# citiususc/veryfasttree

Measured on AMD Instinct MI355X. Metric: profile-ops/sec, higher is better.
Workload: dtype f32; 1 GPU; c4_1M_x200_nt_tophits; n_seqs=1000000, n_pos=200, active_nodes=750000, top_k=2000

## Files before the change

veryfasttree_amd/csrc/vft_api.hip:

```cpp
#include <hip/hip_runtime.h>
#include <csignal>
#include <unistd.h>

#include <cmath>
#include <cstdarg>
#include <cstdio>
#include <cstdlib>
#include <cstring>
#include <new>
#include <algorithm>
#include <utility>
#include <vector>
#include <chrono>

#include "../../include/vft_hip.h"
#include "vft_owned.h"
#include "vft_staging.h"
#define VFT_PAIR_STAGE_CAP 2048
#include "vft_kernels_ml.h"

VFT_ML_HEAVY_INSTANCES(extern)
#include "vft_kernels_ml_long.h"
VFT_ML_LONG_INSTANCES(extern)
#include "vft_kernels_nj.h"
// ... 2231 lines not shown
        c->slots[(size_t) profPos[q]].nPart = (int) gridP;
    }
    a.M.L.mq = nullptr;
    a.M.L.lq = (const uint32_t *) lq;
    a.M.P.mq = (const REAL *) mq;
    a.M.P.lq = nullptr;
    kernel_event(c);
    launch((k_sweep_nt_mixed_multi<REAL, S, S>), dim3((unsigned) (a.nInt + nLeafWGs)), dim3(VFT_WG), 0, c->stream, a);
    kernel_event(c);
    kernel_event(c);
    if (c->timeKernels) c->kevSweeps += 2 * S - 1;
    LAUNCHCHK(c);
    return VFT_OK;
}

static int no_slot(vft_ctx *c) { return fail(c, VFT_ERR_STATE, "the context has no sweep buffers (vft_create failed)"); }

static int sweep_args_ok(vft_ctx *c, int64_t query, int64_t nActive, int32_t k) {
    if (c->slots.empty()) return no_slot(c);
    if (!c->leavesUp) return fail(c, VFT_ERR_STATE, "vft_sweep before vft_upload_leaves");
    if (query < 0 || query >= c->maxnode || nActive < 3 || k < 0 || k > c->hitsCap)
        return fail(c, VFT_ERR_INVALID, "vft_sweep: bad arguments (query %lld, nActive %lld, k %d)", (long long) query,
                    (long long) nActive, (int) k);
    return VFT_OK;
}

extern "C" int vft_sweep(vft_ctx *c, int64_t query, int64_t nActive, int64_t nDiffAllow, double totdiam, int32_t k,
                         void *hits, void *dHitsOut, int64_t *bestJ) {
    if (!c) return VFT_ERR_INVALID;
    if (int r = sweep_args_ok(c, query, nActive, k)) return r;
    if (int r = sweep_one(c, 0, query, nActive, nDiffAllow, totdiam)) return r;
    if (k == 0) return VFT_OK;
    if (bestJ && k < 2) return fail(c, VFT_ERR_INVALID, "vft_sweep: best_j needs k >= 2");
    const int64_t lo = c->shardLo, hi = c->shardHi < c->maxnode ? c->shardHi : c->maxnode;
    int r;
    if (c->cfg.precision == 4) r = run_select<float, vft_hit_f32>(c, 1, &query, lo, hi, k);
    else r = run_select<double, vft_hit_f64>(c, 1, &query, lo, hi, k);
    if (r) return r;
    const size_t hb = (size_t) k * (c->cfg.precision == 4 ? sizeof(vft_hit_f32) : sizeof(vft_hit_f64));
    const vft_ctx::SweepSlotHost &h = c->slots[0];
    if (dHitsOut) HIPCHK(c, hipMemcpyAsync(dHitsOut, h.dRes + sizeof(SelectHeader), hb, hipMemcpyDeviceToDevice, c->stream));
    if (hits) memcpy(hits, h.hRes + sizeof(SelectHeader), hb);
    if (bestJ) *bestJ = (int64_t) ((const SelectHeader *) h.hRes)->bestJ;
    return VFT_OK;
}

struct SeedGroup {
    int pos[4];
    int n;
    bool leaf;
};

extern "C" int vft_sweep_batch(vft_ctx *c, int32_t nSeeds, const int64_t *queries, int64_t nActive, int64_t nDiffAllow,
                               double totdiam, int32_t k, void *hits, void *dHitsOut, int64_t *bestJ) {
    if (!c || !queries || nSeeds < 1 || nSeeds > VFT_MAX_SLOTS || k < 1) return VFT_ERR_INVALID;
    if (bestJ && k < 2) return fail(c, VFT_ERR_INVALID, "vft_sweep_batch: best_j needs k >= 2");
    for (int s = 0; s < nSeeds; s++)
        if (int r = sweep_args_ok(c, queries[s], nActive, k)) return r;
    if (int r = ensure_slots(c, nSeeds)) return r;
    const bool staged = c->cfg.n_codes == 4 && !c->hasDm && nSeeds > 1;
    std::vector<SeedGroup> groups;
    if (staged && !c->noMultiSweep && !(c->maxStamp - nActive > nDiffAllow)) {
        bool fresh = true;
        for (int s = 0; s < nSeeds && fresh; s++) fresh = !((int64_t) c->hNOut[queries[s]] - nActive > nDiffAllow);
        const int maxGroup = c->multiMax ? c->multiMax : 4;
        for (int kind = 0; kind < 2 && fresh; kind++) {
            SeedGroup g{};
            g.leaf = kind == 0;
            int nLeft = 0;
            auto isKind = [&](int s) { return (queries[s] < c->d.nSeqs) == (kind == 0); };
            for (int s = 0; s < nSeeds; s++) nLeft += isKind(s);
            for (int s = 0; s < nSeeds; s++) {
                if (!isKind(s)) continue;
                g.pos[g.n++] = s;
                nLeft--;
                if (g.n == maxGroup || (g.n == 2 && nLeft < 2)) {
                    groups.push_back(g);
                    g.n = 0;
                }
            }
        }
    }
    const int64_t nPosPad = (int64_t) c->d.nChunk * VFT_CHUNK;
    const size_t mqGroupBytes = (size_t) nPosPad * VFT_MQ_STRIDE(4) * c->rs;
    const size_t lqGroupBytes = (size_t) nPosPad * sizeof(uint32_t);
    if (!groups.empty() && !c->mqBuf) {
        OWNCHK(own_group(c, [&]() -> int {
            OWNCHK(own_dev(c, &c->mqBuf, 32 * mqGroupBytes));
            return own_dev(c, &c->lqBuf, 32 * lqGroupBytes);
        }));
        c->mqGroupBytes = mqGroupBytes;
        c->lqGroupBytes = lqGroupBytes;
    }
    if (staged) {
        if (int r = flush_pending(c)) return r;
        std::vector<int> mqGroup((size_t) nSeeds, -1), mqIdx((size_t) nSeeds, 0), mqS((size_t) nSeeds, 0), lqGroup((size_t) nSeeds, -1);
        for (size_t g = 0; g < groups.size(); g++)
            for (int q = 0; q < groups[g].n; q++) {
                (groups[g].leaf ? lqGroup : mqGroup)[(size_t) groups[g].pos[q]] = (int) g;
                mqIdx[(size_t) groups[g].pos[q]] = q;
                mqS[(size_t) groups[g].pos[q]] = groups[g].n;
            }
        Stage st;
        if (int r = st.open(c, (size_t) nSeeds * (c->cfg.precision == 4 ? sizeof(QuerySlot<float>) : sizeof(QuerySlot<double>)), Stage::RING_ONLY)) return r;
        if (c->cfg.precision == 4) {
            for (int s = 0; s < nSeeds; s++) {
                QuerySlot<float> qs;
                qs.node = queries[s];
                qs.q = qbuf_slot<float>(c, s);
                qs.mq = mqGroup[(size_t) s] >= 0 ? (float *) ((char *) c->mqBuf + (size_t) mqGroup[(size_t) s] * c->mqGroupBytes) : nullptr;
                qs.lq = lqGroup[(size_t) s] >= 0 ? (uint32_t *) ((char *) c->lqBuf + (size_t) lqGroup[(size_t) s] * c->lqGroupBytes) : nullptr;
                qs.mqIdx = qs.lqIdx = mqIdx[(size_t) s];
                qs.mqS = qs.lqS = mqS[(size_t) s];
                st.put((size_t) s * sizeof(qs), &qs, sizeof(qs));
            }
            launch((k_extract_query_batch<float, 4>), dim3(cdiv(nPosPad, 256), (unsigned) nSeeds), dim3(256), 0, c->stream, arena<float>(c), st.dev<const QuerySlot<float>>(0));
        } else {
            for (int s = 0; s < nSeeds; s++) {
                QuerySlot<double> qs;
                qs.node = queries[s];
                qs.q = qbuf_slot<double>(c, s);
                qs.mq = mqGroup[(size_t) s] >= 0 ? (double *) ((char *) c->mqBuf + (size_t) mqGroup[(size_t) s] * c->mqGroupBytes) : nullptr;
                qs.lq = lqGroup[(size_t) s] >= 0 ? (uint32_t *) ((char *) c->lqBuf + (size_t) lqGroup[(size_t) s] * c->lqGroupBytes) : nullptr;
                qs.mqIdx = qs.lqIdx = mqIdx[(size_t) s];
                qs.mqS = qs.lqS = mqS[(size_t) s];
                st.put((size_t) s * sizeof(qs), &qs, sizeof(qs));
            }
            launch((k_extract_query_batch<double, 4>), dim3(cdiv(nPosPad, 256), (unsigned) nSeeds), dim3(256), 0, c->stream, arena<double>(c), st.dev<const QuerySlot<double>>(0));
        }
        LAUNCHCHK(c);
    }
    std::vector<char> done((size_t) nSeeds, 0);
    std::vector<char> groupDone(groups.size(), 0);
    if (c->cfg.precision == 4 && !c->noMixedSweep && !groups.empty() && mixed_sweep_fits(c)) {
        size_t gl = 0, gp = 0;
        for (;;) {
            while (gl < groups.size() && !(groups[gl].leaf && groups[gl].n == 4)) gl++;
            while (gp < groups.size() && !(!groups[gp].leaf && groups[gp].n == 4)) gp++;
            if (gl == groups.size() || gp == groups.size()) break;
            const void *mq = (const void *) ((char *) c->mqBuf + gp * c->mqGroupBytes);
            const void *lq = (const void *) ((char *) c->lqBuf + gl * c->lqGroupBytes);
            if (int r = sweep_mixed<float>(c, groups[gl].pos, groups[gp].pos, queries, nActive, nDiffAllow, totdiam, mq, lq)) return r;
            for (int q = 0; q < 4; q++) done[(size_t) groups[gl].pos[q]] = done[(size_t) groups[gp].pos[q]] = 1;
            groupDone[gl++] = groupDone[gp++] = 1;
        }
    }
    for (size_t g = 0; g < groups.size(); g++) {
        if (groupDone[g]) continue;
        const SeedGroup &G = groups[g];
        const void *mq = G.leaf ? nullptr : (const void *) ((char *) c->mqBuf + g * c->mqGroupBytes);
        const void *lq = G.leaf ? (const void *) ((char *) c->lqBuf + g * c->lqGroupBytes) : nullptr;
        int r;
        if (c->cfg.precision == 4) r = G.n == 4 ? sweep_group<float, 4>(c, G.leaf, G.pos, queries, nActive, nDiffAllow, totdiam, mq, lq) : sweep_group<float, 2>(c, G.leaf, G.pos, queries, nActive, nDiffAllow, totdiam, mq, lq);
        else r = G.n == 4 ? sweep_group<double, 4>(c, G.leaf, G.pos, queries, nActive, nDiffAllow, totdiam, mq, lq) : sweep_group<double, 2>(c, G.leaf, G.pos, queries, nActive, nDiffAllow, totdiam, mq, lq);
        if (r) return r;
        for (int q = 0; q < G.n; q++) done[(size_t) G.pos[q]] = 1;
    }
    for (int s = 0; s < nSeeds; s++)
        if (!done[(size_t) s])
            if (int r = sweep_one(c, s, queries[s], nActive, nDiffAllow, totdiam, staged)) return r;
    const int64_t lo = c->shardLo, hi = c->shardHi < c->maxnode ? c->shardHi : c->maxnode;
    int r;
    if (c->cfg.precision == 4) r = run_select<float, vft_hit_f32>(c, nSeeds, queries, lo, hi, k);
    else r = run_select<double, vft_hit_f64>(c, nSeeds, queries, lo, hi, k);
    if (r) return r;
    const size_t hb = (size_t) k * (c->cfg.precision == 4 ? sizeof(vft_hit_f32) : sizeof(vft_hit_f64));
    for (int s = 0; s < nSeeds; s++) {
// ... 1900 lines not shown
```

veryfasttree_amd/csrc/vft_kernels_nj.h:

```cpp
#pragma once
#include "vft_device.h"

#define VFT_WG 256

template <typename REAL>
struct QueryBuf {
    REAL *w;
    uint8_t *code;
    REAL *f;
    uint4 *enc;
    double2 *tab;
};

template <typename REAL>
__device__ __forceinline__ void vft_query_tab(const QueryBuf<REAL> &q, int64_t p, REAL wq, const REAL *f) {
#pragma unroll
    for (int c = 0; c < 5; c++) {
        double2 v = make_double2(0.0, 0.0);
        if (c < 4 && wq > 0) {
            const double wgt = (double) wq;
            const double piece = 1.0 - (double) f[c < 4 ? c : 0];
            v = make_double2(wgt * piece, wgt);
        }
        q.tab[p * 5 + c] = v;
    }
}

template <typename REAL, int NC>
__device__ __forceinline__ void vft_extract_query(const Arena<REAL> &A, int64_t node, const QueryBuf<REAL> &q) {
    const int64_t p = (int64_t) blockIdx.x * blockDim.x + threadIdx.x;
    const int64_t nPosPad = (int64_t) A.d.nChunk * VFT_CHUNK;
    if (p >= nPosPad) return;
    REAL w = 0;
    int code = VFT_NOCODE_;
    REAL f[NC];
#pragma unroll
    for (int k = 0; k < NC; k++) f[k] = 0;
    if (p < A.d.nPos) {
        Col<REAL, NC> c;
        vft_load_col<REAL, NC>(A, node, p, c);
        w = c.w;
        code = c.code;
        if (c.vec) {
#pragma unroll
            for (int k = 0; k < NC; k++) f[k] = c.f[k];
        } else if (NC == 4 && code != VFT_NOCODE_) {
#pragma unroll
            for (int k = 0; k < NC; k++) f[k] = (k == code) ? (REAL) 1 : (REAL) 0;
        }
    }
    q.w[p] = w;
    q.code[p] = (uint8_t) code;
#pragma unroll
    for (int k = 0; k < NC; k++) q.f[p * NC + k] = f[k];
    if (NC == 4) vft_query_tab<REAL>(q, p, w, f);
    if (node < A.d.nSeqs && p < A.d.nChunk) {
        q.enc[p] = A.leafT[vft_leaf_idx(A.d, node >> 6, (int) p, (int) (node & 63))];
    }
}
template <typename REAL, int NC>
__global__ void k_extract_query(Arena<REAL> A, int64_t node, QueryBuf<REAL> q) {
    vft_extract_query<REAL, NC>(A, node, q);
}
#ifdef VFT_NO_PLAIN_COLUMNS
#define VFT_PLAIN_COLUMNS 0
#define VFT_MQ_STRIDE(S) (4 * (S) + 4)
#else
#define VFT_PLAIN_COLUMNS 1
#define VFT_MQ_STRIDE(S) (4 * (S) + 8)
#endif
#ifdef VFT_NO_SEED_CODE_RECORDS
#define VFT_SEED_CODE_RECORDS 0
#else
#define VFT_SEED_CODE_RECORDS 1
#endif
#if defined(VFT_NO_GPR_INDEX_SELECT) || !VFT_SEED_CODE_RECORDS || !VFT_PLAIN_COLUMNS
#define VFT_GPR_INDEX_SELECT 0
#else
#define VFT_GPR_INDEX_SELECT 1
#endif
#if defined(VFT_NO_SHARED_PIECES) || !VFT_GPR_INDEX_SELECT
#define VFT_SHARED_PIECES 0
#else
#define VFT_SHARED_PIECES 1
#endif
template <typename REAL>
struct QuerySlot {
    int64_t node;
    QueryBuf<REAL> q;
    REAL *mq;
    int32_t mqIdx, mqS;
    uint32_t *lq;
    int32_t lqIdx, lqS;
};
template <typename REAL, int NC>
__global__ void k_extract_query_batch(Arena<REAL> A, const QuerySlot<REAL> *qs) {
    const QuerySlot<REAL> &sl = qs[blockIdx.y];
    vft_extract_query<REAL, NC>(A, sl.node, sl.q);
    if (VFT_SEED_CODE_RECORDS && NC == 4 && sl.lq) {
        const int64_t p = (int64_t) blockIdx.x * blockDim.x + threadIdx.x;
        if (p < (int64_t) A.d.nChunk * VFT_CHUNK) {
            uint8_t *dst = (uint8_t *) (sl.lq + p);
            dst[sl.lqIdx] = sl.q.code[p];
            if (sl.lqIdx == 0)
                for (int k = sl.lqS; k < 4; k++) dst[k] = VFT_NOCODE_;
        }
    }
    if (NC == 4 && sl.mq) {
        const int64_t p = (int64_t) blockIdx.x * blockDim.x + threadIdx.x;
        if (p < (int64_t) A.d.nChunk * VFT_CHUNK) {
            REAL *dst = sl.mq + p * VFT_MQ_STRIDE(sl.mqS);
#pragma unroll
            for (int k = 0; k < 4; k++) dst[4 * sl.mqIdx + k] = sl.q.f[p * 4 + k];
            dst[4 * sl.mqS + sl.mqIdx] = sl.q.w[p];
            if (VFT_PLAIN_COLUMNS) ((uint8_t *) (dst + 4 * sl.mqS + 4))[sl.mqIdx] = sl.q.code[p];
        }
    }
}

template <typename REAL, int NC>
__global__ void k_outprofile_as_query(Arena<REAL> A, QueryBuf<REAL> q) {
    const int64_t p = (int64_t) blockIdx.x * blockDim.x + threadIdx.x;
    const int64_t nPosPad = (int64_t) A.d.nChunk * VFT_CHUNK;
    if (p >= nPosPad) return;
    const bool in = p < A.d.nPos;
    q.w[p] = in ? A.outW[p] : (REAL) 0;
    q.code[p] = VFT_NOCODE_;
    REAL f[NC];
#pragma unroll
    for (int k = 0; k < NC; k++) {
        f[k] = in ? A.outF[p * NC + k] : (REAL) 0;
        q.f[p * NC + k] = f[k];
    }
    if (NC == 4) vft_query_tab<REAL>(q, p, in ? A.outW[p] : (REAL) 0, f);
}

struct SweepArgs {
    int64_t query;
    int64_t lo, hi;
    int64_t nActive, nDiffAllow;
    double totdiam;
    int32_t queryIsLeaf;
    int32_t force;
    int32_t nLeafWG;
    int32_t pad;
    int64_t leafEnd;
    int64_t heavyLo;
};

template <typename REAL>
struct SweepOut {
    REAL *dist, *weight, *crit;
    REAL *partMin, *partMax;
};

template <typename REAL, int NWAVES>
__device__ __forceinline__ void vft_block_minmax_n(REAL cmin, REAL cmax, REAL *partMin, REAL *partMax, int part) {
    __shared__ REAL smin[NWAVES], smax[NWAVES];
#pragma unroll
    for (int off = 32; off > 0; off >>= 1) {
        const REAL a = __shfl_xor(cmin, off, 64), b = __shfl_xor(cmax, off, 64);
        cmin = a < cmin ? a : cmin;
        cmax = b > cmax ? b : cmax;
    }
    if ((threadIdx.x & 63) == 0) {
        smin[threadIdx.x >> 6] = cmin;
        smax[threadIdx.x >> 6] = cmax;
    }
    __syncthreads();
    if (threadIdx.x == 0) {
#pragma unroll
        for (int w = 1; w < NWAVES; w++) {
            cmin = smin[w] < cmin ? smin[w] : cmin;
            cmax = smax[w] > cmax ? smax[w] : cmax;
        }
        partMin[part] = cmin;
        partMax[part] = cmax;
    }
}
template <typename REAL>
__device__ __forceinline__ void vft_block_minmax(REAL cmin, REAL cmax, REAL *partMin, REAL *partMax, int part) {
    vft_block_minmax_n<REAL, VFT_WG / 64>(cmin, cmax, partMin, partMax, part);
}

enum { MODE_CRIT = 0, MODE_OUTDIST = 1, MODE_CRIT_LEAFQ = 2 };

__device__ __forceinline__ void vft_seq_counts(const uint4 a, const uint4 b, int &nUse, int &nSame) {
    const uint32_t x = a.x & b.x, y = a.y & b.y, z = a.z & b.z, w = a.w & b.w;
    nUse += __popc(x & 0x10101010u) + __popc(y & 0x10101010u) + __popc(z & 0x10101010u) + __popc(w & 0x10101010u);
    nSame += __popc(x & 0x0F0F0F0Fu) + __popc(y & 0x0F0F0F0Fu) + __popc(z & 0x0F0F0F0Fu) + __popc(w & 0x0F0F0F0Fu);
}

__device__ __forceinline__ void vft_seq_counts_packed(const uint4 a, const uint4 b, uint32_t &cnt) {
    const uint32_t x = a.x & b.x, y = a.y & b.y, z = a.z & b.z, w = a.w & b.w;
    const uint32_t same = __popc(x & 0x0F0F0F0Fu) + __popc(y & 0x0F0F0F0Fu) + __popc(z & 0x0F0F0F0Fu) + __popc(w & 0x0F0F0F0Fu);
    cnt += __popc(x & 0x10101010u) + __popc(y & 0x10101010u) + __popc(z & 0x10101010u) + __popc(w & 0x10101010u);
    cnt += same << 16;
}
// ... 862 lines not shown
        for (int q = 0; q < GC; q++)
#pragma unroll
            for (int bt = 0; bt < NBT; bt++)
#pragma unroll
                for (int sd = 0; sd < S; sd++) {
                    denom[bt][sd] += v[bt][q][sd].y;
                    top[bt][sd] += v[bt][q][sd].x;
                }
    }
}

template <int SL>
struct LeafEncChunk {
    uint4 e[SL > 0 ? SL : 1];
};
template <int SL>
__device__ __forceinline__ void vft_leaf_enc_load(LeafEncChunk<SL> &d, const uint4 *const *enc, int c) {
    typedef uint32_t __attribute__((ext_vector_type(4))) u4_t;
    typedef const __attribute__((address_space(4))) u4_t *cp_t;
#pragma unroll
    for (int q = 0; q < SL; q++) {
        const u4_t v = *((cp_t) enc[q] + c);
        d.e[q] = make_uint4(v.x, v.y, v.z, v.w);
    }
}
template <int NBT, int S, int SL>
__device__ __forceinline__ void vft_leaf_walk_chunk(const double2 *row, const uint4 *t, double (*top)[S], double (*denom)[S],
                                                    const LeafEncChunk<SL> &e, uint32_t (*cnt)[SL > 0 ? SL : 1]) {
    if constexpr (SL > 0) {
#pragma unroll
        for (int bt = 0; bt < NBT; bt++) vft_leaf_table_chunk_multi<1, S, 1>(row, t + bt, top + bt, denom + bt);
        __builtin_amdgcn_sched_barrier(0);
#pragma unroll
        for (int bt = 0; bt < NBT; bt++)
#pragma unroll
            for (int q = 0; q < SL; q++) vft_seq_counts_packed(t[bt], e.e[q], cnt[bt][q]);
    } else {
        vft_leaf_table_chunk_multi<NBT, S>(row, t, top, denom);
    }
}

template <typename REAL, int NBT, int S, int SL = 0>
__device__ __forceinline__ void vft_leaf_table_walk_multi(const Arena<REAL> &A, const MultiLeafQ<REAL, S> &M, double2 *tab, const int64_t *tj,
                                                          double (*top)[S], double (*denom)[S], const uint4 *const *enc = nullptr,
                                                          uint32_t (*cnt)[SL > 0 ? SL : 1] = nullptr) {
    const int tid = threadIdx.x;
    const int64_t nPos = A.d.nPos;
    const uint4 *lp[NBT];
#pragma unroll
    for (int bt = 0; bt < NBT; bt++) lp[bt] = A.leafT + vft_leaf_idx(A.d, tj[bt] >> 6, 0, (int) (tj[bt] & 63));
    for (int64_t p0 = 0; p0 < nPos; p0 += VFT_PTILE_M) {
        __syncthreads();
        {
            const int64_t nTab = ((int64_t) A.d.nChunk * VFT_CHUNK - p0) * 5;
#pragma unroll
            for (int sd = 0; sd < S; sd++)
                for (int e = tid; e < VFT_PTILE_M * 5; e += VFT_WG)
                    tab[sd * (VFT_PTILE_M * 5) + e] = e < nTab ? M.Q[sd].tab[p0 * 5 + e] : make_double2(0.0, 0.0);
        }
        __syncthreads();
        const int c0 = (int) (p0 / VFT_CHUNK);
        const int c1 = (int) (((p0 + VFT_PTILE_M < nPos ? p0 + VFT_PTILE_M : nPos) + VFT_CHUNK - 1) / VFT_CHUNK);
        uint4 ta[NBT], tb[NBT];
        LeafEncChunk<SL> ea, eb;
#pragma unroll
        for (int bt = 0; bt < NBT; bt++) ta[bt] = lp[bt][(int64_t) c0 * VFT_TILE];
        if constexpr (SL > 0) vft_leaf_enc_load<SL>(ea, enc, c0);
        for (int c = c0; c < c1; c += 2) {
            const int cb = c + 1 < c1 ? c + 1 : c, ca = c + 2 < c1 ? c + 2 : c;
#pragma unroll
            for (int bt = 0; bt < NBT; bt++) tb[bt] = lp[bt][(int64_t) cb * VFT_TILE];
            if constexpr (SL > 0) vft_leaf_enc_load<SL>(eb, enc, cb);
            __builtin_amdgcn_sched_barrier(0);
            vft_leaf_walk_chunk<NBT, S, SL>(tab + (int64_t) (c - c0) * VFT_CHUNK * 5, ta, top, denom, ea, cnt);
#pragma unroll
            for (int bt = 0; bt < NBT; bt++) ta[bt] = lp[bt][(int64_t) ca * VFT_TILE];
            if constexpr (SL > 0) vft_leaf_enc_load<SL>(ea, enc, ca);
            __builtin_amdgcn_sched_barrier(0);
            if (c + 1 < c1) vft_leaf_walk_chunk<NBT, S, SL>(tab + (int64_t) (c + 1 - c0) * VFT_CHUNK * 5, tb, top, denom, eb, cnt);
        }
    }
}

template <typename REAL, int S>
__device__ __forceinline__ void vft_leaf_table_wg_multi(const Arena<REAL> &A, const MultiLeafQ<REAL, S> &M, const SweepArgs &s, int64_t base,
                                                        REAL *cmin, REAL *cmax) {
    constexpr int NB = VFT_LEAF_SPAN / VFT_WG, NW = VFT_WG / 64, NBT = 2;
    __shared__ double2 tab[S * VFT_PTILE_M * 5];
    __shared__ unsigned short list[VFT_LEAF_SPAN];
    __shared__ int segCnt[NB * NW];
    const int tid = threadIdx.x, wave = tid >> 6;
    unsigned long long bal[NB];
#pragma unroll
    for (int r = 0; r < NB; r++) {
        const int64_t j = base + r * VFT_WG + tid;
        bool active = false;
        if (j < s.leafEnd) {
            active = A.parent[j] < 0;
            if (!active) {
#pragma unroll
                for (int q = 0; q < S; q++) {
                    M.O[q].dist[j] = (REAL) 1e20;
                    M.O[q].crit[j] = (REAL) 1e20;
                    M.O[q].weight[j] = 0;
                }
            }
        }
        bal[r] = __ballot(active);
        if ((tid & 63) == 0) segCnt[r * NW + wave] = __popcll(bal[r]);
    }
    __syncthreads();
    int nAct = 0, off[NB];
#pragma unroll
    for (int seg = 0; seg < NB * NW; seg++) {
#pragma unroll
        for (int r = 0; r < NB; r++)
            if (seg == r * NW + wave) off[r] = nAct;
        nAct += segCnt[seg];
    }
#pragma unroll
    for (int r = 0; r < NB; r++) {
        const int rank = (int) __builtin_amdgcn_mbcnt_hi((unsigned int) (bal[r] >> 32), __builtin_amdgcn_mbcnt_lo((unsigned int) bal[r], 0u));
        if ((bal[r] >> (tid & 63)) & 1ull) list[off[r] + rank] = (unsigned short) (r * VFT_WG + tid);
    }
    __syncthreads();
    for (int r0 = 0; r0 < nAct; r0 += NBT * VFT_WG) {
        int64_t tj[NBT];
        double top[NBT][S], denom[NBT][S];
#pragma unroll
        for (int bt = 0; bt < NBT; bt++) {
            const int idx = r0 + bt * VFT_WG + tid;
            tj[bt] = base + list[idx < nAct ? idx : 0];
#pragma unroll
            for (int q = 0; q < S; q++) top[bt][q] = denom[bt][q] = 0;
        }
        if (nAct - r0 <= VFT_WG) vft_leaf_table_walk_multi<REAL, 1, S>(A, M, tab, tj, top, denom);
        else vft_leaf_table_walk_multi<REAL, NBT, S>(A, M, tab, tj, top, denom);
#pragma unroll
        for (int bt = 0; bt < NBT; bt++) {
            if (r0 + bt * VFT_WG + tid < nAct) {
#pragma unroll
                for (int q = 0; q < S; q++) {
                    const REAL weight = (REAL) (denom[bt][q] > 0 ? denom[bt][q] : 0.01);
                    const REAL dist = (REAL) (denom[bt][q] > 0 ? top[bt][q] / denom[bt][q] : 1.0);
                    SweepArgs sq = s;
                    sq.query = M.query[q];
                    vft_sweep_finish<REAL, MODE_CRIT>(A, sq, M.O[q], tj[bt], dist, weight, false, cmin[q], cmax[q]);
                }
            }
        }
    }
}

#define VFT_KARG __attribute__((address_space(4)))
template <typename T>
__device__ __forceinline__ const VFT_KARG T *vft_kernarg(size_t off) {
    const VFT_KARG char *p = (const VFT_KARG char *) __builtin_amdgcn_kernarg_segment_ptr() + off;
    asm volatile("" : "+s"(p));
    return (const VFT_KARG T *) p;
}
template <typename REAL>
__device__ __forceinline__ SweepOut<REAL> vft_karg_out(const VFT_KARG SweepOut<REAL> *p) {
    typedef __attribute__((address_space(1))) REAL *gp_t;
    SweepOut<REAL> o;
    o.dist = (REAL *) (gp_t) p->dist;
    o.weight = (REAL *) (gp_t) p->weight;
    o.crit = (REAL *) (gp_t) p->crit;
    o.partMin = (REAL *) (gp_t) p->partMin;
    o.partMax = (REAL *) (gp_t) p->partMax;
    return o;
}
template <typename REAL, int S>
__device__ __forceinline__ void vft_karg_sentinels(const VFT_KARG MultiLeafQ<REAL, S> *M, int64_t j) {
#pragma unroll
    for (int q = 0; q < S; q++) {
        const SweepOut<REAL> O = vft_karg_out<REAL>(&M->O[q]);
        O.dist[j] = (REAL) 1e20;
        O.crit[j] = (REAL) 1e20;
        O.weight[j] = 0;
    }
}
template <typename REAL, int S>
__device__ __forceinline__ void vft_block_minmax_karg(REAL *cmin, REAL *cmax, const VFT_KARG MultiLeafQ<REAL, S> *M, int part,
                                                      REAL (*smin)[VFT_WG / 64], REAL (*smax)[VFT_WG / 64]) {
    constexpr int NW = VFT_WG / 64;
#pragma unroll
    for (int q = 0; q < S; q++) {
#pragma unroll
        for (int off = 32; off > 0; off >>= 1) {
            const REAL a = __shfl_xor(cmin[q], off, 64), b = __shfl_xor(cmax[q], off, 64);
            cmin[q] = a < cmin[q] ? a : cmin[q];
            cmax[q] = b > cmax[q] ? b : cmax[q];
        }
        if ((threadIdx.x & 63) == 0) {
            smin[q][threadIdx.x >> 6] = cmin[q];
            smax[q][threadIdx.x >> 6] = cmax[q];
        }
    }
    __syncthreads();
    if (threadIdx.x < S) {
        const int q = threadIdx.x;
        REAL lo = smin[q][0], hi = smax[q][0];
#pragma unroll
        for (int w = 1; w < NW; w++) {
            lo = smin[q][w] < lo ? smin[q][w] : lo;
            hi = smax[q][w] > hi ? smax[q][w] : hi;
        }
        const SweepOut<REAL> O = vft_karg_out<REAL>(&M->O[q]);
        O.partMin[part] = lo;
        O.partMax[part] = hi;
    }
}

#ifdef VFT_NO_SHARED_LEAF_WALK
#define VFT_SHARED_LEAF_WALK 0
#else
#define VFT_SHARED_LEAF_WALK 1
#endif
#if VFT_SHARED_LEAF_WALK
template <typename REAL, int SL, int SP>
__device__ __forceinline__ void vft_leaf_table_wg_mixed(const Arena<REAL> &A, const MultiLeafQ<REAL, SP> &P, size_t offL, const SweepArgs &s,
                                                        int64_t base, REAL *cminP, REAL *cmaxP, REAL *cminL, REAL *cmaxL) {
    constexpr int NB = VFT_LEAF_SPAN / VFT_WG, NW = VFT_WG / 64, NBT = 2;
    __shared__ double2 tab[SP * VFT_PTILE_M * 5];
    __shared__ unsigned short list[VFT_LEAF_SPAN];
    __shared__ int segCnt[NB * NW];
    const int tid = threadIdx.x, wave = tid >> 6;
    const VFT_KARG MultiLeafQ<REAL, SL> *L0 = vft_kernarg<MultiLeafQ<REAL, SL>>(offL);
    unsigned long long bal[NB];
#pragma unroll
    for (int r = 0; r < NB; r++) {
        const int64_t j = base + r * VFT_WG + tid;
        bool active = false;
        if (j < s.leafEnd) {
            active = A.parent[j] < 0;
            if (!active) {
#pragma unroll
                for (int q = 0; q < SP; q++) {
                    P.O[q].dist[j] = (REAL) 1e20;
                    P.O[q].crit[j] = (REAL) 1e20;
                    P.O[q].weight[j] = 0;
                }
                vft_karg_sentinels<REAL, SL>(L0, j);
            }
        }
        bal[r] = __ballot(active);
        if ((tid & 63) == 0) segCnt[r * NW + wave] = __popcll(bal[r]);
    }
    __syncthreads();
    int nAct = 0, off[NB];
#pragma unroll
    for (int seg = 0; seg < NB * NW; seg++) {
#pragma unroll
        for (int r = 0; r < NB; r++)
            if (seg == r * NW + wave) off[r] = nAct;
        nAct += segCnt[seg];
    }
#pragma unroll
    for (int r = 0; r < NB; r++) {
        const int rank = (int) __builtin_amdgcn_mbcnt_hi((unsigned int) (bal[r] >> 32), __builtin_amdgcn_mbcnt_lo((unsigned int) bal[r], 0u));
        if ((bal[r] >> (tid & 63)) & 1ull) list[off[r] + rank] = (unsigned short) (r * VFT_WG + tid);
    }
    __syncthreads();
    for (int r0 = 0; r0 < nAct; r0 += NBT * VFT_WG) {
        int64_t tj[NBT];
        double top[NBT][SP], denom[NBT][SP];
        uint32_t cnt[NBT][SL];
#pragma unroll
        for (int bt = 0; bt < NBT; bt++) {
            const int idx = r0 + bt * VFT_WG + tid;
            tj[bt] = base + list[idx < nAct ? idx : 0];
#pragma unroll
            for (int q = 0; q < SP; q++) top[bt][q] = denom[bt][q] = 0;
#pragma unroll
            for (int q = 0; q < SL; q++) cnt[bt][q] = 0;
        }
        {
            const VFT_KARG MultiLeafQ<REAL, SL> *L1 = vft_kernarg<MultiLeafQ<REAL, SL>>(offL);
            const uint4 *enc[SL];
#pragma unroll
            for (int q = 0; q < SL; q++) enc[q] = L1->Q[q].enc;
            if (nAct - r0 <= VFT_WG) vft_leaf_table_walk_multi<REAL, 1, SP, SL>(A, P, tab, tj, top, denom, enc, cnt);
            else vft_leaf_table_walk_multi<REAL, NBT, SP, SL>(A, P, tab, tj, top, denom, enc, cnt);
        }
        const VFT_KARG MultiLeafQ<REAL, SL> *Lk = vft_kernarg<MultiLeafQ<REAL, SL>>(offL);
#pragma unroll
        for (int bt = 0; bt < NBT; bt++) {
            const int idx = r0 + bt * VFT_WG + tid;
            tj[bt] = base + list[idx < nAct ? idx : 0];
            if (idx < nAct) {
#pragma unroll
                for (int q = 0; q < SP; q++) {
                    const REAL weight = (REAL) (denom[bt][q] > 0 ? denom[bt][q] : 0.01);
                    const REAL dist = (REAL) (denom[bt][q] > 0 ? top[bt][q] / denom[bt][q] : 1.0);
                    SweepArgs sq = s;
                    sq.query = P.query[q];
                    vft_sweep_finish<REAL, MODE_CRIT>(A, sq, P.O[q], tj[bt], dist, weight, false, cminP[q], cmaxP[q]);
                }
#pragma unroll
                for (int q = 0; q < SL; q++) {
                    const int nUse = (int) (cnt[bt][q] & 0xFFFFu), nSame = (int) (cnt[bt][q] >> 16);
                    const double topq = (double) (nUse - nSame);
                    const REAL weight = (REAL) (double) nUse;
                    const REAL dist = (REAL) (nUse > 0 ? topq / (double) nUse : 1.0);
                    SweepArgs sq = s;
                    sq.query = Lk->query[q];
                    vft_sweep_finish<REAL, MODE_CRIT>(A, sq, vft_karg_out<REAL>(&Lk->O[q]), tj[bt], dist, weight, true, cminL[q], cmaxL[q]);
                }
            }
        }
    }
}
#endif

template <typename REAL, int S>
__global__ __launch_bounds__(VFT_WG, sizeof(REAL) == 4 ? 3 : 2) void k_sweep_nt_profq_multi(Arena<REAL> A, MultiLeafQ<REAL, S> M, SweepArgs s) {
    constexpr int SUB = 8;
    __shared__ REAL smin[S][VFT_WG / 64], smax[S][VFT_WG / 64];
    const int nT = s.nLeafWG, nHeavy = (int) gridDim.x - nT, blk = (int) blockIdx.x;
    REAL cmin[S], cmax[S];
#pragma unroll
    for (int q = 0; q < S; q++) {
        cmin[q] = (REAL) 1e30;
        cmax[q] = (REAL) -1e30;
    }
    if (blk >= nHeavy) {
        const int span = blk - nHeavy;
        vft_leaf_table_wg_multi<REAL, S>(A, M, s, s.lo + (int64_t) span * VFT_LEAF_SPAN, cmin, cmax);
        vft_block_minmax_multi<REAL, S>(cmin, cmax, M.O, span);
        return;
    }
    const int wg = nHeavy - 1 - blk;
    const int64_t j = s.heavyLo + (int64_t) wg * VFT_WG + threadIdx.x;
    const int lane = (int) (j & 63);
    const int64_t tile = j >> 6;
    constexpr size_t offM = (sizeof(Arena<REAL>) + alignof(MultiLeafQ<REAL, S>) - 1) / alignof(MultiLeafQ<REAL, S>) * alignof(MultiLeafQ<REAL, S>);
    const VFT_KARG MultiLeafQ<REAL, S> *M0 = vft_kernarg<MultiLeafQ<REAL, S>>(offM);
    bool work = false;
    if (j < s.hi && !(nT && j < s.leafEnd)) {
        work = A.parent[j] < 0;
        if (!work) vft_karg_sentinels<REAL, S>(M0, j);
    }
    double top[S], denom[S];
#pragma unroll
    for (int q = 0; q < S; q++) top[q] = denom[q] = 0;
    const VFT_KARG MultiLeafQ<REAL, S> *M1 = vft_kernarg<MultiLeafQ<REAL, S>>(offM);
    if (work) {
        const REAL *mq = M1->mq;
        vft_for_column_groups<REAL, SUB>(A, tile, lane, [&](const IntChunkAll<REAL, SUB> &ca, int64_t p0) {
#if VFT_SHARED_PIECES
            if constexpr (sizeof(REAL) == 4 && S == 4) vft_int_chunk_consume_shared<0, S, SUB>(ca, p0, mq, nullptr, top, denom, nullptr, nullptr);
            else
#endif
                vft_int_chunk_consume_prof<REAL, S, SUB, sizeof(REAL) == 4>(ca, p0, mq, top, denom);
            vft_pin_sums<S>(top, denom);
        });
    }
    const VFT_KARG MultiLeafQ<REAL, S> *Mk = vft_kernarg<MultiLeafQ<REAL, S>>(offM);
    if (work) {
#pragma unroll
        for (int q = 0; q < S; q++) {
            const REAL weight = (REAL) (denom[q] > 0 ? denom[q] : 0.01);
            const REAL dist = (REAL) (denom[q] > 0 ? top[q] / denom[q] : 1.0);
            SweepArgs sq = s;
            sq.query = Mk->query[q];
            vft_sweep_finish<REAL, MODE_CRIT>(A, sq, vft_karg_out<REAL>(&Mk->O[q]), j, dist, weight, false, cmin[q], cmax[q]);
// ... 1517 lines not shown
```

Baseline: 17.12 billion profile-ops/s.

## Precompute narrow per-query leaf table in global memory and stage once per workgroup

The query extraction kernel now also writes a precomputed double-precision piece table and weight-denominator array, interleaved across the grouped queries, into extra space appended to the multi-query buffer. The leaf sweep kernels get a new walk that stages this narrow table into LDS, staging only once when the whole padded position range fits in a tile. It uses a software-pipelined per-position loop that loads table entries by code index and reads the weights through scalar loads. This is meant to remove the per-tile on-the-fly table construction and cut LDS footprint and repeated staging. In exchange it uses more global memory per group and adds more register pressure from the pipeline.

Result: no change. 17.21 billion profile-ops/s, median of 2 (+0.5%).

```diff
diff --git a/veryfasttree_amd/csrc/vft_api.hip b/veryfasttree_amd/csrc/vft_api.hip
--- a/veryfasttree_amd/csrc/vft_api.hip
+++ b/veryfasttree_amd/csrc/vft_api.hip
@@ -2337,7 +2337,11 @@
         }
     }
     const int64_t nPosPad = (int64_t) c->d.nChunk * VFT_CHUNK;
+#if VFT_NARROW_LEAF_TABLE
+    const size_t mqGroupBytes = (size_t) nPosPad * VFT_MQ_STRIDE(4) * c->rs + vft_mq_narrow_bytes(nPosPad);
+#else
     const size_t mqGroupBytes = (size_t) nPosPad * VFT_MQ_STRIDE(4) * c->rs;
+#endif
     const size_t lqGroupBytes = (size_t) nPosPad * sizeof(uint32_t);
     if (!groups.empty() && !c->mqBuf) {
         OWNCHK(own_group(c, [&]() -> int {
diff --git a/veryfasttree_amd/csrc/vft_kernels_nj.h b/veryfasttree_amd/csrc/vft_kernels_nj.h
--- a/veryfasttree_amd/csrc/vft_kernels_nj.h
+++ b/veryfasttree_amd/csrc/vft_kernels_nj.h
@@ -83,6 +83,24 @@
 #define VFT_SHARED_PIECES 0
 #else
 #define VFT_SHARED_PIECES 1
+#endif
+#ifdef VFT_NO_NARROW_LEAF_TABLE
+#define VFT_NARROW_LEAF_TABLE 0
+#else
+#define VFT_NARROW_LEAF_TABLE 1
+template <typename REAL>
+__host__ __device__ __forceinline__ size_t vft_mq_record_bytes(int64_t nPosPad) {
+    return (size_t) nPosPad * VFT_MQ_STRIDE(4) * sizeof(REAL);
+}
+__host__ __device__ __forceinline__ size_t vft_mq_narrow_bytes(int64_t nPosPad) { return (size_t) nPosPad * (5 * 4 + 4) * sizeof(double); }
+template <typename REAL>
+__device__ __forceinline__ double *vft_mq_top(const REAL *mq, int64_t nPosPad) {
+    return (double *) ((char *) mq + vft_mq_record_bytes<REAL>(nPosPad));
+}
+template <typename REAL>
+__device__ __forceinline__ double *vft_mq_wd(const REAL *mq, int64_t nPosPad) {
+    return vft_mq_top<REAL>(mq, nPosPad) + nPosPad * (5 * 4);
+}
 #endif
 template <typename REAL>
 struct QuerySlot {
@@ -110,10 +128,31 @@
         const int64_t p = (int64_t) blockIdx.x * blockDim.x + threadIdx.x;
         if (p < (int64_t) A.d.nChunk * VFT_CHUNK) {
             REAL *dst = sl.mq + p * VFT_MQ_STRIDE(sl.mqS);
+#if VFT_NARROW_LEAF_TABLE
+            const int64_t nPosPad = (int64_t) A.d.nChunk * VFT_CHUNK;
+            REAL f[4];
+#pragma unroll
+            for (int k = 0; k < 4; k++) f[k] = sl.q.f[p * 4 + k];
+            const REAL wq = sl.q.w[p];
+            const uint8_t code = sl.q.code[p];
+#pragma unroll
+            for (int k = 0; k < 4; k++) dst[4 * sl.mqIdx + k] = f[k];
+            dst[4 * sl.mqS + sl.mqIdx] = wq;
+            if (VFT_PLAIN_COLUMNS) ((uint8_t *) (dst + 4 * sl.mqS + 4))[sl.mqIdx] = code;
+            double *gt = vft_mq_top<REAL>(sl.mq, nPosPad) + (p * 5) * sl.mqS + sl.mqIdx;
+#pragma unroll
+            for (int k = 0; k < 5; k++) {
+                double v = 0.0;
+                if (k < 4 && wq > 0) v = (double) wq * (1.0 - (double) f[k < 4 ? k : 0]);
+                gt[k * sl.mqS] = v;
+            }
+            vft_mq_wd<REAL>(sl.mq, nPosPad)[p * sl.mqS + sl.mqIdx] = wq > 0 ? (double) wq : 0.0;
+#else
 #pragma unroll
             for (int k = 0; k < 4; k++) dst[4 * sl.mqIdx + k] = sl.q.f[p * 4 + k];
             dst[4 * sl.mqS + sl.mqIdx] = sl.q.w[p];
             if (VFT_PLAIN_COLUMNS) ((uint8_t *) (dst + 4 * sl.mqS + 4))[sl.mqIdx] = sl.q.code[p];
+#endif
         }
     }
 }
@@ -1142,11 +1181,148 @@
     }
 }
 
+#if VFT_NARROW_LEAF_TABLE
+#define VFT_PTILE_N 224
+template <int NBT, int S>
+struct LeafTabPipe {
+    double2 v[NBT][S / 2];
+    double wd[S];
+};
+template <int NBT, int S>
+__device__ __forceinline__ void vft_leaf_pipe_issue(LeafTabPipe<NBT, S> &n, const double *row, const double *wdc, const uint4 *t, int q) {
+    typedef double __attribute__((ext_vector_type(S))) dS_t;
+    typedef const __attribute__((address_space(4))) dS_t *cp_t;
+#pragma unroll
+    for (int bt = 0; bt < NBT; bt++) {
+        const int idx = __ffs((int) (vft_byte(t[bt], q) | 0x10u)) - 1;
+        const double2 *e = (const double2 *) (row + (q * 5 + idx) * S);
+#pragma unroll
+        for (int h = 0; h < S / 2; h++) n.v[bt][h] = e[h];
+    }
+    const dS_t w = *((cp_t) (wdc + q * S));
+#pragma unroll
+    for (int sd = 0; sd < S; sd++) n.wd[sd] = w[sd];
+}
+template <int NBT, int S>
+__device__ __forceinline__ void vft_leaf_table_chunk_narrow(LeafTabPipe<NBT, S> &cur, const double *row, const double *wdc, const uint4 *t,
+                                                            const double *rowN, const double *wdN, const uint4 *tN, double (*top)[S],
+                                                            double (*denom)[S]) {
+#pragma unroll
+    for (int q = 0; q < VFT_CHUNK; q++) {
+#pragma unroll
+        for (int sd = 0; sd < S; sd++) asm volatile("" : "+s"(cur.wd[sd]));
+#pragma unroll
+        for (int bt = 0; bt < NBT; bt++)
+#pragma unroll
+            for (int h = 0; h < S / 2; h++) asm volatile("" : "+v"(cur.v[bt][h].x), "+v"(cur.v[bt][h].y));
+        LeafTabPipe<NBT, S> nxt;
+        if (q + 1 < VFT_CHUNK) vft_leaf_pipe_issue<NBT, S>(nxt, row, wdc, t, q + 1);
+        else vft_leaf_pipe_issue<NBT, S>(nxt, rowN, wdN, tN, 0);
+        __builtin_amdgcn_sched_barrier(0);
+#pragma unroll
+        for (int bt = 0; bt < NBT; bt++) {
+            const uint32_t w = q < 8 ? (q < 4 ? t[bt].x : t[bt].y) : (q < 12 ? t[bt].z : t[bt].w);
+            const int32_t m = (int32_t) (w << (27 - 8 * (q & 3))) >> 31;
+            const double ng = __hiloint2double((int) ((uint32_t) m & 0x3FF00000u), 0);
+#pragma unroll
+            for (int sd = 0; sd < S; sd++) {
+                denom[bt][sd] = __builtin_fma(cur.wd[sd], ng, denom[bt][sd]);
+                top[bt][sd] += (sd & 1) ? cur.v[bt][sd / 2].y : cur.v[bt][sd / 2].x;
+            }
+        }
+        __builtin_amdgcn_sched_barrier(0);
+        cur = nxt;
+    }
+}
+template <typename REAL, int S>
+__device__ __forceinline__ void vft_leaf_table_stage_narrow(const Arena<REAL> &A, const REAL *mq, double2 *tab, int64_t p0) {
+    const int64_t nPosPad = (int64_t) A.d.nChunk * VFT_CHUNK;
+    const double2 *src = (const double2 *) (vft_mq_top<REAL>(mq, nPosPad) + p0 * 5 * S);
+    const int64_t nTab = (nPosPad - p0) * 5 * (S / 2);
+    for (int e = threadIdx.x; e < VFT_PTILE_N * 5 * (S / 2); e += VFT_WG) tab[e] = e < nTab ? src[e] : make_double2(0.0, 0.0);
+}
+template <typename REAL, int NBT, int S, int SL>
+__device__ __forceinline__ void vft_leaf_table_tile_narrow(const Arena<REAL> &A, const REAL *mq, const double2 *tab, int64_t p0, const uint4 *const *lp,
+                                                           double (*top)[S], double (*denom)[S], const uint4 *const *enc,
+                                                           uint32_t (*cnt)[SL > 0 ? SL : 1]) {
+    const int64_t nPos = A.d.nPos;
+    const double *wd = vft_mq_wd<REAL>(mq, (int64_t) A.d.nChunk * VFT_CHUNK);
+    const double *row0 = (const double *) tab;
+    const int c0 = (int) (p0 / VFT_CHUNK);
+    const int c1 = (int) (((p0 + VFT_PTILE_N < nPos ? p0 + VFT_PTILE_N : nPos) + VFT_CHUNK - 1) / VFT_CHUNK);
+    uint4 ta[NBT], tb[NBT];
+    LeafEncChunk<SL> ea, eb;
+    LeafTabPipe<NBT, S> pipe;
+#pragma unroll
+    for (int bt = 0; bt < NBT; bt++) ta[bt] = lp[bt][(int64_t) c0 * VFT_TILE];
+    if constexpr (SL > 0) vft_leaf_enc_load<SL>(ea, enc, c0);
+    vft_leaf_pipe_issue<NBT, S>(pipe, row0, wd + (int64_t) c0 * VFT_CHUNK * S, ta, 0);
+    for (int c = c0; c < c1; c += 2) {
+        const int cb = c + 1 < c1 ? c + 1 : c, ca = c + 2 < c1 ? c + 2 : c;
+#pragma unroll
+        for (int bt = 0; bt < NBT; bt++) tb[bt] = lp[bt][(int64_t) cb * VFT_TILE];
+        if constexpr (SL > 0) vft_leaf_enc_load<SL>(eb, enc, cb);
+        __builtin_amdgcn_sched_barrier(0);
+        vft_leaf_table_chunk_narrow<NBT, S>(pipe, row0 + (int64_t) (c - c0) * VFT_CHUNK * 5 * S, wd + (int64_t) c * VFT_CHUNK * S, ta,
+                                            row0 + (int64_t) (cb - c0) * VFT_CHUNK * 5 * S, wd + (int64_t) cb * VFT_CHUNK * S, tb, top, denom);
+        if constexpr (SL > 0) {
+            __builtin_amdgcn_sched_barrier(0);
+#pragma unroll
+            for (int bt = 0; bt < NBT; bt++)
+#pragma unroll
+                for (int q = 0; q < SL; q++) vft_seq_counts_packed(ta[bt], ea.e[q], cnt[bt][q]);
+        }
+#pragma unroll
+        for (int bt = 0; bt < NBT; bt++) ta[bt] = lp[bt][(int64_t) ca * VFT_TILE];
+        if constexpr (SL > 0) vft_leaf_enc_load<SL>(ea, enc, ca);
+        __builtin_amdgcn_sched_barrier(0);
+        if (c + 1 < c1) {
+            vft_leaf_table_chunk_narrow<NBT, S>(pipe, row0 + (int64_t) (c + 1 - c0) * VFT_CHUNK * 5 * S, wd + (int64_t) (c + 1) * VFT_CHUNK * S, tb,
+                                                row0 + (int64_t) (ca - c0) * VFT_CHUNK * 5 * S, wd + (int64_t) ca * VFT_CHUNK * S, ta, top, denom);
+            if constexpr (SL > 0) {
+                __builtin_amdgcn_sched_barrier(0);
+#pragma unroll
+                for (int bt = 0; bt < NBT; bt++)
+#pragma unroll
+                    for (int q = 0; q < SL; q++) vft_seq_counts_packed(tb[bt], eb.e[q], cnt[bt][q]);
+            }
+        }
+    }
+}
+template <typename REAL, int NBT, int S, int SL = 0>
+__device__ __forceinline__ void vft_leaf_table_walk_narrow(const Arena<REAL> &A, const REAL *mq, double2 *tab, const int64_t *tj, bool staged,
+                                                           double (*top)[S], double (*denom)[S], const uint4 *const *enc = nullptr,
+                                                           uint32_t (*cnt)[SL > 0 ? SL : 1] = nullptr) {
+    const uint4 *lp[NBT];
+#pragma unroll
+    for (int bt = 0; bt < NBT; bt++) lp[bt] = A.leafT + vft_leaf_idx(A.d, tj[bt] >> 6, 0, (int) (tj[bt] & 63));
+    for (int64_t p0 = 0; p0 < A.d.nPos; p0 += VFT_PTILE_N) {
+        if (!staged) {
+            __syncthreads();
+            vft_leaf_table_stage_narrow<REAL, S>(A, mq, tab, p0);
+            __syncthreads();
+        }
+        vft_leaf_table_tile_narrow<REAL, NBT, S, SL>(A, mq, tab, p0, lp, top, denom, enc, cnt);
+    }
+}
+template <typename REAL, int S>
+__device__ __forceinline__ bool vft_leaf_table_stage_once(const Arena<REAL> &A, const REAL *mq, double2 *tab) {
+    if ((int64_t) A.d.nChunk * VFT_CHUNK > VFT_PTILE_N) return false;
+    vft_leaf_table_stage_narrow<REAL, S>(A, mq, tab, 0);
+    __syncthreads();
+    return true;
+}
+#endif
+
 template <typename REAL, int S>
 __device__ __forceinline__ void vft_leaf_table_wg_multi(const Arena<REAL> &A, const MultiLeafQ<REAL, S> &M, const SweepArgs &s, int64_t base,
                                                         REAL *cmin, REAL *cmax) {
     constexpr int NB = VFT_LEAF_SPAN / VFT_WG, NW = VFT_WG / 64, NBT = 2;
+#if VFT_NARROW_LEAF_TABLE
+    __shared__ double2 tab[(S / 2) * VFT_PTILE_N * 5];
+#else
     __shared__ double2 tab[S * VFT_PTILE_M * 5];
+#endif
     __shared__ unsigned short list[VFT_LEAF_SPAN];
     __shared__ int segCnt[NB * NW];
     const int tid = threadIdx.x, wave = tid >> 6;
@@ -1184,6 +1360,9 @@
         if ((bal[r] >> (tid & 63)) & 1ull) list[off[r] + rank] = (unsigned short) (r * VFT_WG + tid);
     }
     __syncthreads();
+#if VFT_NARROW_LEAF_TABLE
+    const bool staged = nAct > 0 && vft_leaf_table_stage_once<REAL, S>(A, M.mq, tab);
+#endif
     for (int r0 = 0; r0 < nAct; r0 += NBT * VFT_WG) {
         int64_t tj[NBT];
         double top[NBT][S], denom[NBT][S];
@@ -1194,8 +1373,13 @@
 #pragma unroll
             for (int q = 0; q < S; q++) top[bt][q] = denom[bt][q] = 0;
         }
+#if VFT_NARROW_LEAF_TABLE
+        if (nAct - r0 <= VFT_WG) vft_leaf_table_walk_narrow<REAL, 1, S>(A, M.mq, tab, tj, staged, top, denom);
+        else vft_leaf_table_walk_narrow<REAL, NBT, S>(A, M.mq, tab, tj, staged, top, denom);
+#else
         if (nAct - r0 <= VFT_WG) vft_leaf_table_walk_multi<REAL, 1, S>(A, M, tab, tj, top, denom);
         else vft_leaf_table_walk_multi<REAL, NBT, S>(A, M, tab, tj, top, denom);
+#endif
 #pragma unroll
         for (int bt = 0; bt < NBT; bt++) {
             if (r0 + bt * VFT_WG + tid < nAct) {
@@ -1282,7 +1466,11 @@
 __device__ __forceinline__ void vft_leaf_table_wg_mixed(const Arena<REAL> &A, const MultiLeafQ<REAL, SP> &P, size_t offL, const SweepArgs &s,
                                                         int64_t base, REAL *cminP, REAL *cmaxP, REAL *cminL, REAL *cmaxL) {
     constexpr int NB = VFT_LEAF_SPAN / VFT_WG, NW = VFT_WG / 64, NBT = 2;
+#if VFT_NARROW_LEAF_TABLE
+    __shared__ double2 tab[(SP / 2) * VFT_PTILE_N * 5];
+#else
     __shared__ double2 tab[SP * VFT_PTILE_M * 5];
+#endif
     __shared__ unsigned short list[VFT_LEAF_SPAN];
     __shared__ int segCnt[NB * NW];
     const int tid = threadIdx.x, wave = tid >> 6;
@@ -1322,6 +1510,9 @@
         if ((bal[r] >> (tid & 63)) & 1ull) list[off[r] + rank] = (unsigned short) (r * VFT_WG + tid);
     }
     __syncthreads();
+#if VFT_NARROW_LEAF_TABLE
+    const bool staged = nAct > 0 && vft_leaf_table_stage_once<REAL, SP>(A, P.mq, tab);
+#endif
     for (int r0 = 0; r0 < nAct; r0 += NBT * VFT_WG) {
         int64_t tj[NBT];
         double top[NBT][SP], denom[NBT][SP];
@@ -1340,8 +1531,13 @@
             const uint4 *enc[SL];
 #pragma unroll
             for (int q = 0; q < SL; q++) enc[q] = L1->Q[q].enc;
+#if VFT_NARROW_LEAF_TABLE
+            if (nAct - r0 <= VFT_WG) vft_leaf_table_walk_narrow<REAL, 1, SP, SL>(A, P.mq, tab, tj, staged, top, denom, enc, cnt);
+            else vft_leaf_table_walk_narrow<REAL, NBT, SP, SL>(A, P.mq, tab, tj, staged, top, denom, enc, cnt);
+#else
             if (nAct - r0 <= VFT_WG) vft_leaf_table_walk_multi<REAL, 1, SP, SL>(A, P, tab, tj, top, denom, enc, cnt);
             else vft_leaf_table_walk_multi<REAL, NBT, SP, SL>(A, P, tab, tj, top, denom, enc, cnt);
+#endif
         }
         const VFT_KARG MultiLeafQ<REAL, SL> *Lk = vft_kernarg<MultiLeafQ<REAL, SL>>(offL);
 #pragma unroll
```
